# jabirali/bodge

Hardware: AMD Instinct MI355X
Metric: Chebyshev SpMV steps/s + achieved HBM GB/s, 4N×4N BdG H; free_energy wall-time (higher is better)
Workload: dtype f64

## Files before the change

bodge_amd/backend.py:

```python

from __future__ import annotations

import ctypes as C
import os

import numpy as np

LIBRARY_PATH = os.environ.get(
    "BODGE_AMD_LIBRARY", os.path.join(os.path.dirname(os.path.abspath(__file__)), "csrc", "libbodge_hip.so")
)

VEC_RADEMACHER = 0
VEC_Z4 = 1

_f64p = C.POINTER(C.c_double)
_i32p = C.POINTER(C.c_int32)
_i64p = C.POINTER(C.c_int64)
_u8p = C.POINTER(C.c_uint8)
_handle = C.c_void_p


class Perf(C.Structure):
    _fields_ = [
        ("kernel_ms", C.c_double),
        ("launches", C.c_int64),
        ("vector_steps", C.c_int64),
        ("bytes_per_launch", C.c_double),
        ("lanes_per_row", C.c_int32),
        ("vectors_per_launch", C.c_int32),
        ("grid", C.c_int32),
        ("lds_bytes", C.c_int32),
        ("pipelined", C.c_int32),
        ("real_arithmetic", C.c_int32),
        ("strip_rows", C.c_int32),
        ("ph_packed", C.c_int32),
        ("dict_blocks", C.c_int32),
        ("steps_per_launch", C.c_int32),
        ("rolling", C.c_int32),
        ("dict_skipped", C.c_int32),
        ("onsite_streamed", C.c_int32),
        ("streams", C.c_int32),
        ("bytes_moved", C.c_double),
        ("window_ms", C.c_double),
        ("sweeps", C.c_int64),
        ("persistent", C.c_int32),
        ("groups_per_launch", C.c_int32),
        ("clenshaw", C.c_int32),
        ("green", C.c_int32),
        ("green_ranges", C.c_int32),
        ("green_local", C.c_int32),
        ("apply", C.c_int32),
    ]


SIGNATURES = {
    "bdg_last_error": (C.c_char_p, []),
    "bdg_version": (C.c_char_p, []),
    "bdg_device_count": (C.c_int, [C.POINTER(C.c_int)]),
    "bdg_create": (C.c_int, [C.c_int, C.c_int64, C.c_int64, _i32p, _i32p, _f64p, C.POINTER(_handle)]),
    "bdg_create_slab": (
        C.c_int,
        [C.c_int, C.c_int64, C.c_int64, C.c_int64, _i32p, _i32p, _f64p, C.c_int64, C.POINTER(_handle)],
    ),
    "bdg_slab_set_exchange": (C.c_int, [_handle, _handle, C.c_int32, _i32p, _i64p, _i64p, _i64p, _i64p]),
    "bdg_group_create": (C.c_int, [C.POINTER(_handle), C.c_int32, C.POINTER(_handle)]),
    "bdg_group_destroy": (C.c_int, [_handle]),
    "bdg_group_dots_random": (
        C.c_int,
        [_handle, C.c_double, C.c_int32, C.c_int32, C.c_uint64, C.c_uint64, C.c_int32, _f64p, _f64p],
    ),
    "bdg_group_dots_unit": (C.c_int, [_handle, C.c_double, C.c_int32, C.c_int32, _i64p, _f64p, _f64p]),
    "bdg_destroy": (C.c_int, [_handle]),
    "bdg_spmv": (C.c_int, [_handle, _f64p, _f64p]),
    "bdg_cheb_dots_random": (
        C.c_int,
        [_handle, C.c_double, C.c_int32, C.c_int32, C.c_uint64, C.c_uint64, C.c_int32, _f64p, _f64p],
    ),
    "bdg_cheb_dots_unit": (C.c_int, [_handle, C.c_double, C.c_int32, C.c_int32, _i64p, _f64p, _f64p]),
    "bdg_cheb_moments": (
        C.c_int,
        [_handle, _handle, C.c_double, C.c_int32, C.c_int32, C.c_uint64, C.c_uint64, C.c_int32, _f64p],
    ),
    "bdg_fermi_blocks": (
        C.c_int,
# ... 127 lines not shown
```

bodge_amd/csrc/core.hpp:

```cpp
#pragma once

namespace {

thread_local std::string g_error;

int fail(int code, const char* fmt, ...) {
    char buf[512];
    va_list ap;
    va_start(ap, fmt);
    vsnprintf(buf, sizeof buf, fmt, ap);
    va_end(ap);
    g_error = buf;
    return code;
}

#define HIP_TRY(expr)                                                                   \
    do {                                                                                \
        hipError_t err__ = (expr);                                                      \
        if (err__ != hipSuccess)                                                        \
            return fail(err__ == hipErrorOutOfMemory ? BDG_ENOMEM : BDG_EDEVICE,        \
                        "%s failed: %s (%s:%d)", #expr, hipGetErrorString(err__),       \
                        __FILE__, __LINE__);                                            \
    } while (0)

// ... 118 lines not shown
    bool group_peer_access = true;
    hipStream_t comm_stream = nullptr;
    hipEvent_t ev_step_done = nullptr, ev_halo_ready = nullptr;
    DeviceBuffer<int> tiles_interior, tiles_boundary;
    int split_rows_per_tile = 0, n_interior = 0, n_boundary = 0;
    void* lanczos = nullptr;
    int max_row_blocks = 0;
    int64_t bandwidth = 0;
    int num_cus = 0;
    size_t lds_per_cu = 0;
    int lanes_override = 0;
    DeviceBuffer<int> indptr, indices;
    DeviceBuffer<double2> blocks;
    DeviceBuffer<double2> packed[4];
    bool is_real = false;
    bool is_ph = false;
    double gershgorin = 0.0;
    int n_unique = 0;
    int dict_skipped = 0;
    bool onsite_streamed = false;
    DeviceBuffer<double2> onsite[2];
    bool bonds_streamed = false;
    DeviceBuffer<double2> site_records[2];
    int site_records_plane[2] = {0, 0};
    DeviceBuffer<int> dict_ids;
    DeviceBuffer<unsigned> dict_ell;
    int dict_ell_words = 0;
    DeviceBuffer<int> dict_diagonal;
    DeviceBuffer<double2> dict_full;
    DeviceBuffer<double2> dict_table[4];
    DeviceBuffer<uint2> stencil;
    int stencil_state = 0;
    bool stencil_wrap_p = false, stencil_wrap_x = false;
    double* host_dots = nullptr;
    size_t host_dots_count = 0;
    int shape[3] = {0, 0, 0};
    struct TileOrder {
        int rows_per_tile = 0, strip_rows = 0;
        DeviceBuffer<int> ids;
    };
    std::vector<std::unique_ptr<TileOrder>> tile_orders;
    bdg_perf perf{};
};

namespace {
inline void release_side_sets(bdg_system* sys) {
    for (auto& side : sys->side_sets) {
        if (side->stream) (void)hipStreamSynchronize(side->stream);
        side->release_set();
    }
    sys->side_sets.clear();
}
}

struct bdg_comm {
    int device = 0;
    int n_ranks = 1, rank = 0;
    ncclComm_t comm = nullptr;
    hipStream_t stream = nullptr;
    DeviceBuffer<double> scratch;
};

struct bdg_group {
    std::vector<bdg_system*> members;
    std::vector<hipEvent_t> packed, copied;
    std::vector<hipEvent_t> stepped[2];
// ... 2 lines not shown
```

bodge_amd/csrc/plans.hpp:

```cpp
#pragma once

namespace {

using StepKernel = void (*)(bdg::StepArgs);

using bdg::ComplexMode;
using bdg::ComplexPHMode;
using bdg::RealMode;
using bdg::RealPHMode;

struct ModeInfo {
    int id;
    bool real, ph;
    int per_lane;
    int stride;
    double block_bytes;
    double entry_bytes;
};

ModeInfo mode_info(bool real, bool ph) {
    if (real && ph) return {3, true, true, RealPHMode::kVec, RealPHMode::kBlockStride, 100.0, 96.0};
    if (real) return {1, true, false, RealMode::kVec, RealMode::kBlockStride, 132.0, 96.0};
    if (ph) return {2, false, true, ComplexPHMode::kVec, ComplexPHMode::kBlockStride, 196.0, 192.0};
    return {0, false, false, ComplexMode::kVec, ComplexMode::kBlockStride, 260.0, 192.0};
// ... 388 lines not shown
}

SweepKernel sweep3_gen_kernel(const ModeInfo& mode, int lanes) {
    switch (mode.id) {
        case 1: return sweep3_gen_kernel_for<RealMode>(lanes);
        case 2: return sweep3_gen_kernel_for<ComplexPHMode>(lanes);
        case 3: return sweep3_gen_kernel_for<RealPHMode>(lanes);
    }
    return sweep3_gen_kernel_for<ComplexMode>(lanes);
}

template <typename Mode, int RL, int OS, int WAVES>
SweepKernel sweep3_streamed_pick(bool reverse, bool gen) {
    return gen ? bdg::cheb_sweep3<Mode, RL, false, true, OS, WAVES>
               : reverse ? bdg::cheb_sweep3<Mode, RL, true, false, OS, WAVES> : bdg::cheb_sweep3<Mode, RL, false, false, OS, WAVES>;
}
SweepKernel sweep3_streamed_kernel(const ModeInfo& mode, int lanes, int waves, bool reverse, bool gen, bool bonds = false) {
    if (!mode.ph) return nullptr;
    if (bonds) {
        if (mode.real) return lanes == 4 && waves == 4 ? sweep3_streamed_pick<RealPHMode, 4, 2, 4>(reverse, gen) : nullptr;
        return lanes == 4 && waves == 7 ? sweep3_streamed_pick<ComplexPHMode, 4, 2, 7>(reverse, gen) : nullptr;
    }
    if (mode.real) {
        if (lanes == 4 && waves == 4) return sweep3_streamed_pick<RealPHMode, 4, 1, 4>(reverse, gen);
        if (lanes == 2 && waves == 4) return sweep3_streamed_pick<RealPHMode, 2, 1, 4>(reverse, gen);
        if (lanes == 2 && waves == 7) return sweep3_streamed_pick<RealPHMode, 2, 1, 7>(reverse, gen);
        return nullptr;
    }
    if (lanes == 4 && waves == 4) return sweep3_streamed_pick<ComplexPHMode, 4, 1, 4>(reverse, gen);
    if (lanes == 2 && waves == 7) return sweep3_streamed_pick<ComplexPHMode, 2, 1, 7>(reverse, gen);
    return nullptr;
}

size_t sweep3_lds_bytes(const bdg_system* sys, const ModeInfo& mode, int lanes, int waves) {
    size_t bytes = (size_t)sys->n_unique * mode.stride * sizeof(double2) +
                   (size_t)sys->n_unique * (mode.id == 0 ? 4 : mode.id == 3 ? 1 : 2) * sizeof(double2) +
                   (size_t)sys->n_unique * (mode.id == 3 ? RealPHMode::kSingletSlots : 0) * sizeof(double2);
    size_t per_wave = (size_t)3 * bdg::kWave * 4 * sizeof(double2);
    if (sys->onsite_streamed) {
        const int stride = sys->bonds_streamed ? (mode.real ? bdg::sweep3_record_stride<RealPHMode, 2>() : bdg::sweep3_record_stride<ComplexPHMode, 2>())
                                               : (mode.real ? bdg::sweep3_record_stride<RealPHMode, 1>() : bdg::sweep3_record_stride<ComplexPHMode, 1>());
        per_wave += (size_t)3 * (bdg::kWave / lanes) * stride * sizeof(double2);
    }
    return bytes + (size_t)waves * per_wave;
}

int streamed_waves_for(const bdg_system* sys, const ModeInfo& mode, int lanes) {
    if (!sys->onsite_streamed || !mode.ph) return 0;
    int best = 0, best_resident = 0;
    for (int waves : {4, 7}) {
        if (!sweep3_streamed_kernel(mode, lanes, waves, false, false, sys->bonds_streamed)) continue;
        const size_t lds = sweep3_lds_bytes(sys, mode, lanes, waves);
        if (lds > sys->lds_per_cu) continue;
        const int resident = waves * (int)std::min<size_t>(waves > 4 ? 1 : 2, sys->lds_per_cu / lds);
        if (resident > best_resident) best = waves, best_resident = resident;
    }
    return best;
}

SweepKernel sweep3_kernel(const ModeInfo& mode, int lanes, bool reverse) {
    switch (mode.id) {
        case 1: return sweep3_kernel_for<RealMode>(lanes, reverse);
        case 2: return sweep3_kernel_for<ComplexPHMode>(lanes, reverse);
        case 3: return sweep3_kernel_for<RealPHMode>(lanes, reverse);
    }
    return sweep3_kernel_for<ComplexMode>(lanes, reverse);
}

using MarchKernel = void (*)(bdg::MarchArgs);
template <typename Mode>
MarchKernel march3_kernel_for(int lanes) {
    switch (lanes) {
        case 2: return bdg::cheb_march3<Mode, 2, 0>;
        case 4: return bdg::cheb_march3<Mode, 4, 0>;
    }
    return nullptr;
}
MarchKernel march3_kernel(const ModeInfo& mode, int lanes, bool streamed, bool bonds) {
    if (streamed) {
        if (!mode.ph || lanes != 4) return nullptr;
        if (bonds) return mode.real ? bdg::cheb_march3<RealPHMode, 4, 2> : nullptr;
        return mode.real ? bdg::cheb_march3<RealPHMode, 4, 1> : bdg::cheb_march3<ComplexPHMode, 4, 1>;
    }
    switch (mode.id) {
        case 1: return march3_kernel_for<RealMode>(lanes);
        case 2: return march3_kernel_for<ComplexPHMode>(lanes);
        case 3: return march3_kernel_for<RealPHMode>(lanes);
    }
    return march3_kernel_for<ComplexMode>(lanes);
}

struct SweepPlan {
    int lanes = bdg::kSweepLanes;
    int depth = 2;
    SweepKernel kernel = nullptr, kernel_reverse = nullptr;
    SweepKernel kernel_gen = nullptr;
    MarchKernel march = nullptr;
    int march_grid = 0;
    int grid = 0;
    int wg_waves = bdg::kSweepWaves;
    size_t lds_bytes = 0;
    bdg::SweepArgs args{};
    int waves = 0;
    int whole_segs = 1;
    int segments_for(int planes) const {
        if (planes >= args.lx) return whole_segs;
        return std::max(1, std::min(choose_segments(args.n_cols, planes, waves, 2 * depth, 2), planes / 2));
    }
};

constexpr int64_t kSweepMinSites = 150000;
constexpr int64_t kSweepMinSitesWide = 90000;
constexpr int64_t kRollMinSites = 600000;
constexpr int64_t kSweepTwoLaneSites = 250000;

int ensure_stencil(bdg_system* sys, int* kind) {
    *kind = 0;
    const int64_t plane = (int64_t)sys->shape[1] * sys->shape[2];
    if (sys->stencil_state == 0) {
        sys->stencil_state = -1;
        sys->stencil_lo_base = sys->stencil_hi_base = -1;
        const bool shaped = plane >= 2 * bdg::kSweepOwned && sys->shape[0] >= 8 &&
                            (int64_t)sys->shape[0] * plane == sys->nb;
        const bool three_d = sys->shape[1] > 1 && sys->shape[2] > 1;
        bool slab_ok = sys->ncols == sys->nb;
        if (!slab_ok && shaped && three_d) {
            slab_ok = true;
            const int64_t lx = sys->shape[0];
            int64_t lo = -1, hi = -1;
            for (const auto& ref : sys->halo_refs) {
                const int64_t x = ref.first / plane, p = ref.first % plane, base = (int64_t)ref.second - p;
                if (x == 0 && (lo < 0 || lo == base)) lo = base;
                else if (x == lx - 1 && (hi < 0 || hi == base)) hi = base;
                else slab_ok = false;
            }
            for (int64_t base : {lo, hi})
                if (base >= 0 && (base < sys->nb || base + plane > sys->ncols)) slab_ok = false;
            if (slab_ok) {
                sys->stencil_lo_base = (int)lo;
                sys->stencil_hi_base = (int)hi;
            }
        }
        if (shaped && slab_ok && sys->n_unique > 0 && sys->n_unique < (int)bdg::kNoBlock &&
            sys->max_row_blocks <= (three_d ? 7 : 5) && sys->nnzb > 0 && !(three_d && sys->onsite_streamed)) {
            if (int rc = sys->stencil.reserve((size_t)sys->nb)) return rc;
            DeviceBuffer<int> bad;
            if (int rc = bad.reserve(3)) return rc;
            int host_bad[3] = {1, 0, 0};
            auto body = [&]() -> int {
                HIP_TRY(hipMemsetAsync(bad.ptr, 0, 3 * sizeof(int), sys->stream));
                const unsigned grid = (unsigned)std::min<int64_t>(4096, (sys->nb + 255) / 256);
                if (three_d)
                    bdg::build_stencil3<<<grid, 256, 0, sys->stream>>>(sys->indptr.ptr, sys->dict_ids.ptr,
                                                                        sys->dict_diagonal.ptr, (int)sys->nb, (int)plane,
                                                                        sys->shape[2], sys->stencil_lo_base, sys->stencil_hi_base,
                                                                        sys->stencil.ptr, bad.ptr);
                else
                    bdg::build_stencil<<<grid, 256, 0, sys->stream>>>(sys->indptr.ptr, sys->dict_ids.ptr,
                                                                       sys->dict_diagonal.ptr, (int)sys->nb, (int)plane,
                                                                       sys->bonds_streamed ? 2 : sys->onsite_streamed ? 1 : 0,
                                                                       sys->stencil.ptr, bad.ptr);
                HIP_TRY(hipGetLastError());
                HIP_TRY(hipMemcpyAsync(host_bad, bad.ptr, 3 * sizeof(int), hipMemcpyDeviceToHost, sys->stream));
                HIP_TRY(hipStreamSynchronize(sys->stream));
                return BDG_OK;
            };
            const int rc = body();
            bad.release();
            if (rc) return rc;
            if (host_bad[0] == 0) {
                sys->stencil_state = three_d ? 2 : 1;
                sys->stencil_wrap_p = host_bad[1] != 0;
                sys->stencil_wrap_x = host_bad[2] != 0;
            } else {
                sys->stencil.release();
            }
        }
    }
    *kind = std::max(0, sys->stencil_state);
    return BDG_OK;
}

inline int64_t plane_sites(const bdg_system* sys) { return (int64_t)sys->shape[1] * sys->shape[2]; }

int sweep_wanted(bdg_system* sys, bool col_scalars, int* kind, bool wide_call = false) {
    *kind = 0;
    const char* env = knob::raw("BODGE_AMD_SWEEP");
    if ((env && env[0] == '0') || col_scalars) return BDG_OK;
    const bool slab = !sys->peers.empty() || sys->ncols != sys->nb;
    if (slab && (sys->slab_comm || sys->group_rows == 0)) return BDG_OK;
    const bool forced = env && env[0] == '1';
    const int64_t lattice_rows = std::max(sys->nb, sys->group_rows);
    const int64_t min_2d = wide_call ? kSweepMinSitesWide : kSweepMinSites;
    if (!forced && lattice_rows < std::min(min_2d, kRollMinSites)) return BDG_OK;
    const char* dict_env = knob::raw("BODGE_AMD_DICT");
    if (dict_env && dict_env[0] == '0') return BDG_OK;
    if (int rc = ensure_stencil(sys, kind)) return rc;
    if (slab && *kind != 2) *kind = 0;
    if (!forced && lattice_rows < (*kind == 2 ? kRollMinSites : min_2d)) *kind = 0;
    return BDG_OK;
}

int make_sweep_plan(bdg_system* sys, const ModeInfo& mode, int lanes, int depth, SweepPlan* plan, int share = 1) {
    plan->lanes = lanes;
    plan->depth = depth;
    const bool streamed = sys->onsite_streamed, bonds = sys->bonds_streamed;
    const int wg_waves = streamed ? streamed_waves_for(sys, mode, lanes) : bdg::kSweepWaves;
    if (streamed && (depth != 3 || wg_waves == 0))
        return fail(BDG_EINVAL, "streamed on-site blocks need the three-step sweep, particle-hole packed blocks and a lane count whose ring of records fits the LDS (%d lanes do not)", lanes);
    plan->wg_waves = wg_waves;
    plan->kernel = streamed ? sweep3_streamed_kernel(mode, lanes, wg_waves, false, false, bonds)
                            : depth == 3 ? sweep3_kernel(mode, lanes, false) : sweep_kernel(mode, lanes, false);
    plan->kernel_reverse = streamed ? sweep3_streamed_kernel(mode, lanes, wg_waves, true, false, bonds)
                                    : depth == 3 ? sweep3_kernel(mode, lanes, true) : sweep_kernel(mode, lanes, true);
    plan->kernel_gen = streamed ? sweep3_streamed_kernel(mode, lanes, wg_waves, false, true, bonds) : depth == 3 ? sweep3_gen_kernel(mode, lanes) : nullptr;
    if (!plan->kernel) return fail(BDG_EINVAL, "the sweep kernel has 1, 2 or 4 lanes per site, not %d", lanes);
    const size_t table = (size_t)sys->n_unique * mode.stride * sizeof(double2);
    if (table > table_limit(sys)) return fail(BDG_EINVAL, "block table too large for the sweep kernel");
    if (depth == 3) {
        plan->lds_bytes = sweep3_lds_bytes(sys, mode, lanes, wg_waves);
    } else {
        plan->lds_bytes = table + (size_t)bdg::kSweepWaves * depth * bdg::kWave * 4 * sizeof(double2);
    }
    if (plan->lds_bytes > 64 * 1024)
        for (SweepKernel k : {plan->kernel, plan->kernel_reverse, plan->kernel_gen})
            if (k) HIP_TRY(hipFuncSetAttribute(reinterpret_cast<const void*>(k), hipFuncAttributeMaxDynamicSharedMemorySize,
                                        (int)plan->lds_bytes));
    plan->march = depth == 3 && wg_waves == bdg::kWavesPerBlock &&
                          (size_t)sys->ncols * lanes * 4 * sizeof(double2) < ((size_t)1 << 31) && sys->ncols == sys->nb
                      ? march3_kernel(mode, lanes, streamed, bonds) : nullptr;
    if (plan->march && plan->lds_bytes > 64 * 1024)
        HIP_TRY(hipFuncSetAttribute(reinterpret_cast<const void*>(plan->march), hipFuncAttributeMaxDynamicSharedMemorySize,
                                    (int)plan->lds_bytes));
    int per_cu = 0;
    HIP_TRY(hipOccupancyMaxActiveBlocksPerMultiprocessor(&per_cu, reinterpret_cast<const void*>(plan->kernel),
                                                         wg_waves * bdg::kWave, plan->lds_bytes));
    per_cu = std::max(1, std::min(per_cu, wg_waves > 4 ? 1 : 2 * bdg::kWavesPerBlock / bdg::kSweepWaves));
    if (const char* cap = knob::raw("BODGE_AMD_BLOCKS_PER_CU")) per_cu = std::max(1, atoi(cap));
    const int64_t plane = (int64_t)sys->shape[1] * sys->shape[2];
    bdg::SweepArgs& a = plan->args;
    a = bdg::SweepArgs{};
    a.stencil = sys->stencil.ptr;
    if (int rc = ensure_dict_table(sys, mode, &a.dict_table)) return rc;
    if (bonds) {
        if (int rc = ensure_site_records(sys, (int)plane, mode.real, &a.onsite)) return rc;
    } else if (streamed) {
        if (int rc = ensure_onsite(sys, mode.real, &a.onsite)) return rc;
    }
    a.n_unique = sys->n_unique;
    a.nb = (int)sys->nb;
    a.plane = (int)plane;
    a.lx = sys->shape[0];
    const int owned = depth == 3 ? bdg::sweep3_owned(lanes) : bdg::sweep_owned(lanes);
// ... 194 lines not shown
```

bodge_amd/csrc/recurrence.hpp:

```cpp
#pragma once

namespace {

constexpr int kMarchAborted = -77;

struct Batch {
    bdg_system* sys = nullptr;
    StreamSet* ss = nullptr;
    int next = 0;
    int stream_share = 1;
    StepPlan plan;
    bdg::StepArgs args{};
    bool real = false;
    bool alternate = false;
    int64_t band_lo = -1, band_hi = -1;
    int plane_lo = -1, plane_hi = -1;
    ModeInfo mode{};
    int rl = 0, rv = 0, n_active = 0, n_steps = 0, chunk = 1, strip_rows = 0;
    size_t width = 0, per_step = 0, vec_count = 0;
    double scale = 1.0;
    double2* cur = nullptr;
    double2* prev = nullptr;
    float kernel_ms = 0.f;
    int n_chunks = 0;
// ... 575 lines not shown
            sys->march_seen[0] = 0;
            (void)hipMemsetAsync(sys->march_gave_up.ptr, 0, sizeof(unsigned), sys->stream);
            (void)hipStreamSynchronize(sys->stream);
            sys->march_off = true;
            return kMarchAborted;
        }
        const double* host = sys->host_dots + (size_t)slot * host_stride;
        if (march_follower) n_chunks = 0;
        for (int c = 0; c < n_chunks; ++c) {
            float ms = 0.f;
            HIP_TRY(hipEventElapsedTime(&ms, ss->ev_pool[2 * (ev_base + c)], ss->ev_pool[2 * (ev_base + c) + 1]));
            kernel_ms += ms;
        }
        for (int n = 0; n < n_steps; ++n)
            for (int r = 0; r < n_active; ++r) {
                double& d = d_out[(size_t)n * ld + col0 + r];
                double& e = e_out[(size_t)n * ld + col0 + r];
                const double dv = host[(size_t)n * width + 2 * r], ev = host[(size_t)n * width + 2 * r + 1];
                d = accumulate ? d + dv : dv;
                e = accumulate ? e + ev : ev;
            }
        bdg_perf& p = sys->perf;
        if (first_batch) p = bdg_perf{};
        p.kernel_ms += kernel_ms;
        p.launches += sweep ? n_launches : n_steps;
        p.bytes_moved += bytes_moved;
        p.window_ms = p.kernel_ms;
        p.streams = 1;
        p.vector_steps += (int64_t)n_steps * n_active;
        p.bytes_per_launch = sweep  ? sweep_bytes(sys, mode, rl)
                             : roll ? roll_bytes(sys, mode, rl)
                                    : algorithmic_bytes(sys, rv, mode, plan.dictionary);
        p.steps_per_launch = sweep ? splan.depth : 1;
        p.persistent = march ? 1 : 0;
        p.sweeps += march ? sweeps_counted : sweep ? n_launches : 0;
        p.rolling = roll ? 1 : 0;
        p.dict_skipped = sys->dict_skipped;
        p.onsite_streamed = sweep && sys->onsite_streamed ? (sys->bonds_streamed ? 2 : 1) : 0;
        p.lanes_per_row = rl;
        p.vectors_per_launch = rv;
        p.real_arithmetic = real ? 1 : 0;
        p.ph_packed = mode.ph ? 1 : 0;
        p.dict_blocks = plan.dictionary ? sys->n_unique : 0;
        p.strip_rows = strip_rows;
        p.grid = march ? splan.march_grid : launch_grid;
        p.lds_bytes = (int32_t)(sweep ? splan.lds_bytes : roll ? rplan.lds_bytes : plan.lds_footprint);
        p.pipelined = plan.pipelined ? 1 : 0;
        return BDG_OK;
    }
};

int march_run(Batch* const* list, int count) {
    Batch& lead = *list[0];
    bdg_system* sys = lead.sys;
    HIP_TRY(hipSetDevice(sys->device));
    hipStream_t st = lead.ss->stream;
    const bdg::SweepArgs& geo = lead.splan.args;
    const int units = geo.n_cols * geo.n_segs;
    for (int g = 0; g < count; ++g) {
        Batch& b = *list[g];
        if (!b.march || b.next != lead.next || b.n_steps != lead.n_steps || b.rl != lead.rl || b.mode.id != lead.mode.id ||
            b.splan.args.n_segs != geo.n_segs || b.chunk != lead.chunk)
            return fail(BDG_EINVAL, "lane groups of one persistent launch must share plan and progress");
        b.march_follower = g > 0;
        b.work_stream = st;
        if (g > 0) {
// ... 441 lines not shown
```

bodge_amd/csrc/sweep.hpp:

```cpp
#pragma once

#include "kernels.hpp"

namespace bdg {

constexpr int kSweepLanes = 4;
constexpr int kSweepSlots = kWave / kSweepLanes;
constexpr int kSweepOwned = kSweepSlots - 4;
constexpr int sweep_owned(int rl) { return kWave / rl - 4; }
constexpr unsigned kNoBlock = 0xFFu;

struct SweepArgs {
    const uint2* stencil;
    const void* dict_table;
    int n_unique;
    const double2* onsite;
    const double2* cur;
    const double2* prev;
    double2* out1;
    double2* out2;
    double* partial1;
    double* partial2;
    double coef1, coef2;
    int nb;
// ... 21 lines not shown
    const int lx = nb / plane;
    for (int i = blockIdx.x * blockDim.x + threadIdx.x; i < nb; i += gridDim.x * blockDim.x) {
        unsigned id[5] = {kNoBlock, kNoBlock, kNoBlock, kNoBlock, kNoBlock};
        unsigned mask = 0;
        const int p = i % plane, x = i / plane;
        bool ok = true;
        for (int k = indptr[i]; k < indptr[i + 1]; ++k) {
            const unsigned w = (unsigned)words[k];
            const int off = (int)(w & 0xFFFFFFu) - i;
            int slot = -1;
            if (off == -plane) slot = 0;
            else if (off == -1 && p >= 1) slot = 1;
            else if (off == 0) slot = 2;
            else if (off == 1 && p <= plane - 2) slot = 3;
            else if (off == plane) slot = 4;
            else if (off == plane - 1 && p == 0) {
                slot = 1;
                atomicOr(bad + 1, 1);
            } else if (off == -(plane - 1) && p == plane - 1) {
                slot = 3;
                atomicOr(bad + 1, 1);
            } else if (off == (lx - 1) * plane && x == 0) {
                slot = 0;
                atomicOr(bad + 2, 1);
            } else if (off == -(lx - 1) * plane && x == lx - 1) {
                slot = 4;
                atomicOr(bad + 2, 1);
            }
            if (slot < 0 || (w >> 24) == kNoBlock) ok = false;
            else if (onsite_streamed == 2 || (onsite_streamed && slot == 2)) id[slot] = 0;
            else {
                id[slot] = w >> 24;
                if (diagonal[w >> 24] == 1) mask |= 1u << slot;
                if (diagonal[w >> 24] == 2 && slot != 2) mask |= 32u << slot;
            }
        }
        if (!ok) atomicOr(bad, 1);
        stencil[i] = make_uint2(id[0] | (id[1] << 8) | (id[2] << 16) | (id[3] << 24), id[4] | (mask << 8));
    }
}

__global__ void pack_site_records(const int* __restrict__ indptr, const int* __restrict__ indices,
                                  const double2* __restrict__ blocks, int nb, int plane, int real_out, double2* __restrict__ out) {
    const int lx = nb / plane;
    for (int i = blockIdx.x * blockDim.x + threadIdx.x; i < nb; i += gridDim.x * blockDim.x) {
        const double2 zero = make_double2(0.0, 0.0);
        double2 rec[14] = {zero, zero, zero, zero, zero, zero, zero, zero, zero, zero, zero, zero, zero, zero};
        const int p = i % plane, x = i / plane;
        for (int k = indptr[i]; k < indptr[i + 1]; ++k) {
            const double2* blk = blocks + (size_t)k * 16;
            const int off = indices[k] - i;
            int slot = -1;
            if (off == -plane) slot = 0;
            else if (off == -1 && p >= 1) slot = 1;
            else if (off == 0) slot = 2;
            else if (off == 1 && p <= plane - 2) slot = 3;
            else if (off == plane) slot = 4;
            else if (off == plane - 1 && p == 0) slot = 1;
            else if (off == -(plane - 1) && p == plane - 1) slot = 3;
            else if (off == (lx - 1) * plane && x == 0) slot = 0;
            else if (off == -(lx - 1) * plane && x == lx - 1) slot = 4;
            const int bond = slot < 2 ? slot : slot - 1;
            if (slot == 2 && real_out) {
                rec[0] = make_double2(blk[0].x, blk[1].x);
                rec[1] = make_double2(blk[5].x, 0.0);
                rec[2] = make_double2(blk[2].x, blk[3].x);
// ... 288 lines not shown
#define BDG_SWEEP_BUFFER_OPS 1
#endif
__device__ __forceinline__ __amdgpu_buffer_rsrc_t sweep_plane_rsrc(const void* buf, size_t byte_offset, int bytes) {
    const uint64_t base = reinterpret_cast<uint64_t>(buf) + byte_offset;
    const uint32_t lo = __builtin_amdgcn_readfirstlane((uint32_t)base), hi = __builtin_amdgcn_readfirstlane((uint32_t)(base >> 32));
    return __builtin_amdgcn_make_buffer_rsrc(reinterpret_cast<void*>(((uint64_t)hi << 32) | lo), 0, bytes, kRawBufferFlags);
}

struct Sweep3Gen {
    uint64_t key0 = 0, key1 = 0;
    bool on0 = false, on1 = false;
};
template <typename Mode>
__device__ inline Sweep3Gen sweep3_gen_keys(uint64_t seed, uint64_t first_id, int active, int r) {
    Sweep3Gen g;
    const int v0 = Mode::kVec == 2 ? 2 * r : r;
    g.on0 = v0 < active;
    g.on1 = Mode::kVec == 2 && v0 + 1 < active;
    g.key0 = vector_key(seed, first_id + v0);
    g.key1 = vector_key(seed, first_id + v0 + 1);
    return g;
}

struct Sweep3Task {
    const double2* cur;
    const double2* prev;
    double2* out1;
    double2* out2;
    double coef1;
    int steps;
    int discard;
};

template <typename Mode, int RL, bool GEN, int OS, bool WT>
__device__ __forceinline__ void sweep3_unit(const SweepArgs& a, const Sweep3Task& t, const Sweep3Lds& w, const Sweep3Gen& gen, int lane,
                                            int seg, int col, bool rev, double (&dot1)[4], double (&dot2)[4], double (&dot3)[4]) {
    constexpr int SLOTS = kWave / RL;
    constexpr int OWNED3 = SLOTS - 6;
    constexpr int STRIDE = Mode::kBlockStride;
    constexpr int RING = sweep3_ring_slots<Mode, OS>(SLOTS);
    constexpr int RSTRIDE = sweep3_record_stride<Mode, OS>();
    constexpr int DSL = Mode::kDiagSlots;
    const int s = lane / RL;
    const int r = lane % RL;
    double2* const lds = w.table;
    double2* const diag = w.diag;
    [[maybe_unused]] double2* const singlet = w.singlet;
    double2* const row_0 = w.row_0;
    double2* const row_1 = w.row_1;
    double2* const row_2 = w.row_2;
    [[maybe_unused]] double2* const os_ring = w.os_ring;
    const double2 zero = make_double2(0.0, 0.0);
    const size_t nb = (size_t)a.nb;
    const int steps = t.steps;
    const bool nt_prev = a.stream & 1, nt_cur = a.stream & 4;
    [[maybe_unused]] const bool nt_store = a.stream & 2;
    [[maybe_unused]] const uint64_t gen_key0 = gen.key0, gen_key1 = gen.key1;
    [[maybe_unused]] const bool gen_on0 = gen.on0, gen_on1 = gen.on1;

    const int x0 = a.x_lo + (int)(((int64_t)(a.x_hi - a.x_lo) * seg) / a.n_segs);
    const int x1 = a.x_lo + (int)(((int64_t)(a.x_hi - a.x_lo) * (seg + 1)) / a.n_segs);
    const int p = col * OWNED3 - 3 + s;
    const bool inside = p >= 0 && p < a.plane;
    const bool valid = inside || a.wrap_p;
    const int pw = inside ? p : ((p % a.plane) + a.plane) % a.plane;
    const bool ok1 = valid && s >= 1 && s <= SLOTS - 2;
    const bool ok2 = valid && s >= 2 && s <= SLOTS - 3;
// ... 138 lines not shown
        double2 x[4];
        [[maybe_unused]] const double2* rec = nullptr;
        if constexpr (OS != 0) rec = ring_entry(kk) + s * RSTRIDE;
        auto bond = [&](int slot, const double2 v[4]) {
            if constexpr (OS == 2) {
                if (id_of(w, slot) != kNoBlock) Mode::mac_bond(acc, rec + Mode::kOnsiteSlots + Mode::kBondSlots * (slot < 2 ? slot : slot - 1), v);
            } else {
                mac(w, slot, v, acc);
            }
        };
        if (rev) bond(0, after);
        else bond(0, before);
        if (id_of(w, 1) != kNoBlock) {
#pragma unroll
            for (int be = 0; be < 4; ++be) x[be] = row[SHARE_SLOT(lane - RL, be)];
            bond(1, x);
        }
        if constexpr (OS != 0) {
#if !(BDG_OS_EXPERIMENT & 4)
            if (id_of(w, 2) != kNoBlock) Mode::mac_onsite(acc, rec, mid);
#endif
        } else {
            mac(w, 2, mid, acc);
        }
        if (id_of(w, 3) != kNoBlock) {
#pragma unroll
            for (int be = 0; be < 4; ++be) x[be] = row[SHARE_SLOT(lane + RL, be)];
            bond(3, x);
        }
        if (rev) bond(4, before);
        else bond(4, after);
    };

    constexpr int OSL = OS != 0 ? (SLOTS * sweep3_onsite_pieces<Mode, OS>() + kWave - 1) / kWave : 1;
    [[maybe_unused]] auto load_onsite = [&](int k, bool wanted, double2 out[OSL]) {
        if constexpr (OS != 0) {
            constexpr int PIECES = sweep3_record_slots<Mode, OS>();
            k = ring(act(k));
#pragma unroll
            for (int j = 0; j < OSL; ++j) {
                const int e = lane + j * kWave, slot = e / PIECES, part = e - slot * PIECES;
                const int pe = col * OWNED3 - 3 + slot;
                const bool in_e = pe >= 0 && pe < a.plane;
                const int pwe = in_e ? pe : ((pe % a.plane) + a.plane) % a.plane;
                out[j] = zero;
                {
                    const bool there = wanted && k >= 0 && k < a.lx;
                    const __amdgpu_buffer_rsrc_t rsrc = sweep_plane_rsrc(a.onsite, there ? (size_t)k * a.plane * PIECES * sizeof(double2) : 0,
                                                                         there ? a.plane * PIECES * (int)sizeof(double2) : 0);
                    const int piece_bytes = slot < SLOTS && (in_e || a.wrap_p) ? (pwe * PIECES + part) * (int)sizeof(double2) : kBufferOutOfRange;
                    out[j] = __builtin_bit_cast(double2, __builtin_amdgcn_raw_buffer_load_b128(rsrc, piece_bytes, 0, 0));
                }
            }
        }
    };
    [[maybe_unused]] auto put_onsite = [&](int kk, const double2 v[OSL]) {
        if constexpr (OS != 0) {
            constexpr int PIECES = sweep3_record_slots<Mode, OS>();
            double2* dst = ring_entry(kk);
#pragma unroll
            for (int j = 0; j < OSL; ++j) {
                const int e = lane + j * kWave, slot = e / PIECES, part = e - slot * PIECES;
                if (slot < SLOTS) dst[slot * RSTRIDE + part] = v[j];
            }
        }
    };

    double2 cn_m[4], buf_a[4], buf_b[4], pv[4], c1_m[4], c2_m[4];
    cur_plane(k_first - 1, valid, cn_m);
    cur_plane(k_first, valid, buf_a);
    cur_plane(k_first + 1, valid, buf_b);
    load_plane(t.prev, nt_prev, k_first, !GEN && ok1 && t.prev != nullptr, pv);
    uint2 ids_0 = load_ids(k_first), ids_1 = make_uint2(0xFFFFFFFFu, 0xFFu), ids_2 = ids_1;
#pragma unroll
    for (int al = 0; al < 4; ++al) c1_m[al] = c2_m[al] = zero;
    put_own(row_1, c1_m);
    put_own(row_2, c1_m);
    if constexpr (OS != 0) {
        double2 first_os[OSL];
        load_onsite(k_first, true, first_os);
        put_onsite(k_first, first_os);
    }

    auto iterate = [&](int k, double2 (&centre)[4], const double2 (&after)[4]) {
        const bool more = k < k_last;
        const uint2 nx_ids = load_ids(k + 1, more);
        put_own(row_0, centre);
        wave_sync();
        cur_plane(k + 2, valid && more, centre);

        double2 new1[4], new2[4];
#pragma unroll
        for (int al = 0; al < 4; ++al) new1[al] = new2[al] = zero;
        if (ok1 && in_lattice(k)) {
            double2 acc[4], mid[4];
#pragma unroll
            for (int al = 0; al < 4; ++al) acc[al] = zero;
            own_of(row_0, mid);
            apply(ids_0, cn_m, row_0, mid, after, acc, k);
#pragma unroll
            for (int al = 0; al < 4; ++al) {
                new1[al].x = fma(t.coef1, acc[al].x, -pv[al].x);
                new1[al].y = fma(t.coef1, acc[al].y, -pv[al].y);
            }
            if (owned && k >= x0 && k < x1) {
#pragma unroll
                for (int al = 0; al < 4; ++al) Mode::dots(dot1, mid[al], new1[al]);
                if (steps == 1) store_plane(t.out2, k, new1);
                if (steps == 2) store_plane(t.out1, k, new1);
            }
        }
        load_plane(t.prev, nt_prev, k + 1, !GEN && ok1 && more && t.prev != nullptr, pv);

        if (steps >= 2 && ok2 && in_lattice(k - 1) && k - 1 >= x0 - (steps - 2) && k - 1 < x1 + (steps - 2)) {
            double2 acc[4], mid[4];
#pragma unroll
            for (int al = 0; al < 4; ++al) acc[al] = zero;
            own_of(row_1, mid);
            apply(ids_1, c1_m, row_1, mid, new1, acc, k - 1);
#pragma unroll
            for (int al = 0; al < 4; ++al) {
                new2[al].x = fma(a.coef2, acc[al].x, -cn_m[al].x);
                new2[al].y = fma(a.coef2, acc[al].y, -cn_m[al].y);
            }
            if (owned && k - 1 >= x0 && k - 1 < x1) {
#pragma unroll
                for (int al = 0; al < 4; ++al) Mode::dots(dot2, mid[al], new2[al]);
                if (steps == 2) store_plane(t.out2, k - 1, new2);
                if (steps == 3) store_plane(t.out1, k - 1, new2);
            }
        }

        [[maybe_unused]] double2 nx_os[OSL];
#if BDG_OS_EXPERIMENT & 1
        load_onsite(k + 1, false, nx_os);
#else
        load_onsite(k + 1, more, nx_os);
#endif

        if (steps >= 3 && owned && k - 2 >= x0 && k - 2 < x1) {
            double2 acc[4], mid[4], new3[4];
#pragma unroll
            for (int al = 0; al < 4; ++al) acc[al] = zero;
            own_of(row_2, mid);
            apply(ids_2, c2_m, row_2, mid, new2, acc, k - 2);
#pragma unroll
            for (int al = 0; al < 4; ++al) {
                new3[al].x = fma(a.coef2, acc[al].x, -c1_m[al].x);
                new3[al].y = fma(a.coef2, acc[al].y, -c1_m[al].y);
                Mode::dots(dot3, mid[al], new3[al]);
            }
            store_plane(t.out2, k - 2, new3);
        }

        wave_sync();
        own_of(row_0, cn_m);
        own_of(row_1, c1_m);
        own_of(row_2, c2_m);
        wave_sync();
        put_own(row_1, new1);
        put_own(row_2, new2);
#if !(BDG_OS_EXPERIMENT & 2)
        put_onsite(k + 1, nx_os);
#endif
        ids_2 = ids_1;
        ids_1 = ids_0;
        ids_0 = nx_ids;
    };
    for (int k = k_first; k <= k_last; k += 2) {
        iterate(k, buf_a, buf_b);
        if (k + 1 <= k_last) iterate(k + 1, buf_b, buf_a);
    }
}

template <typename Mode, int OS, int THREADS = kBlockThreads>
__device__ inline Sweep3Lds sweep3_stage_lds(double2* lds, const SweepArgs& a, int slots, int wave) {
    constexpr int SPB = Mode::kSlotsPerBlock;
    constexpr int STRIDE = Mode::kBlockStride;
    constexpr int DSL = Mode::kDiagSlots;
    const int ring = sweep3_ring_slots<Mode, OS>(slots);
    const double2* table = static_cast<const double2*>(a.dict_table);
    for (int e = threadIdx.x; e < a.n_unique * SPB; e += THREADS)
        lds[(e / SPB) * STRIDE + (e % SPB)] = table[e];
    constexpr int SSL = Mode::kSingletSlots;
    Sweep3Lds w;
    w.table = lds;
    w.diag = lds + a.n_unique * STRIDE;
    w.singlet = w.diag + a.n_unique * DSL;
    w.row_0 = w.singlet + a.n_unique * SSL + wave * (3 * kWave * 4 + ring);
    w.row_1 = w.row_0 + kWave * 4;
    w.row_2 = w.row_1 + kWave * 4;
    w.os_ring = w.row_2 + kWave * 4;
    __syncthreads();
    for (int id = threadIdx.x; id < a.n_unique; id += THREADS) {
        Mode::pack_diag(w.diag + id * DSL, lds + id * STRIDE);
        if constexpr (SSL > 0) Mode::pack_singlet(w.singlet + id * SSL, lds + id * STRIDE);
    }
    __syncthreads();
    return w;
}

template <typename Mode, int RL, bool REV, bool GEN = false, int OS = 0, int WAVES = kWavesPerBlock>
__global__ __launch_bounds__(WAVES * kWave, WAVES > 4 ? 1 : 2) void cheb_sweep3(SweepArgs a) {
    extern __shared__ double2 lds[];
    const int lane = threadIdx.x & (kWave - 1);
    const int wave = __builtin_amdgcn_readfirstlane(threadIdx.x / kWave);
    const Sweep3Lds w = sweep3_stage_lds<Mode, OS, WAVES * kWave>(lds, a, kWave / RL, wave);

    const int n_units = a.n_cols * a.n_segs;
    const int xcd = blockIdx.x & 7;
    const int u_lo = (int)(((int64_t)n_units * xcd) >> 3);
    const int u_hi = (int)(((int64_t)n_units * (xcd + 1)) >> 3);
    const int waves_per_xcd = (gridDim.x >> 3) * WAVES;

    double dot1[4] = {0.0, 0.0, 0.0, 0.0}, dot2[4] = {0.0, 0.0, 0.0, 0.0}, dot3[4] = {0.0, 0.0, 0.0, 0.0};
    Sweep3Gen gen;
    if constexpr (GEN) gen = sweep3_gen_keys<Mode>(a.gen_seed, a.gen_first_id, a.gen_active, lane % RL);

    const Sweep3Task task{a.cur, a.prev, a.out1, a.out2, a.coef1, a.steps, a.discard};
    for (int u = u_lo + (int)(blockIdx.x >> 3) * WAVES + wave; u < u_hi; u += waves_per_xcd) {
        const int seg = u / a.n_cols, col = u - seg * a.n_cols;
        const bool rev = REV != (bool)(a.zigzag & seg & 1);
        sweep3_unit<Mode, RL, GEN, OS, false>(a, task, w, gen, lane, seg, col, rev, dot1, dot2, dot3);
    }

    const int steps = a.steps;
    __syncthreads();
    sweep_reduce_dots<Mode, RL, WAVES>(dot1, reinterpret_cast<double*>(lds), a.partial1, lane, wave);
    if (steps >= 2) {
        __syncthreads();
        sweep_reduce_dots<Mode, RL, WAVES>(dot2, reinterpret_cast<double*>(lds), a.partial2, lane, wave);
    }
    if (steps >= 3) {
        __syncthreads();
        sweep_reduce_dots<Mode, RL, WAVES>(dot3, reinterpret_cast<double*>(lds), a.partial3, lane, wave);
    }
}

constexpr int kMarchGroups = 4;
constexpr int kMarchMaxLevels = 24;
constexpr int kMarchCounterWords = 32;

struct MarchGroup {
    double2* buf[4];
    double* partial;
    unsigned long long gen_first_id;
    int gen_active;
    int pad;
};

struct MarchArgs {
    SweepArgs base;
    MarchGroup group[kMarchGroups];
    int n_groups;
    int n_levels;
    int last_steps;
    int discard_last;
    int first_is_start;
    int gen;
    int rev0;
    int units;
    unsigned long long per_step;
    unsigned* sync;
    unsigned flags_at;
    unsigned timeout_ticks;
    unsigned* gave_up;
    int fixed;
    int debug;
    int poll_sleep;
// ... 384 lines not shown
```

include/bodge_hip.h:

```cpp
#ifndef BODGE_HIP_H
#define BODGE_HIP_H

#include <stdint.h>

#ifdef __cplusplus
extern "C" {
#endif

#define BDG_OK 0
#define BDG_EINVAL (-1)
#define BDG_EDEVICE (-2)
#define BDG_ENOMEM (-3)
#define BDG_ELIBRARY (-4)

#define BDG_VEC_RADEMACHER 0
#define BDG_VEC_Z4 1

typedef struct bdg_system bdg_system;
typedef struct bdg_comm bdg_comm;
typedef struct bdg_group bdg_group;

typedef struct bdg_perf {
    double kernel_ms;
    int64_t launches;
    int64_t vector_steps;
    double bytes_per_launch;
    int32_t lanes_per_row;
    int32_t vectors_per_launch;
    int32_t grid;
    int32_t lds_bytes;
    int32_t pipelined;
    int32_t real_arithmetic;
    int32_t strip_rows;
    int32_t ph_packed;
    int32_t dict_blocks;
    int32_t steps_per_launch;
    int32_t rolling;
    int32_t dict_skipped;
    int32_t onsite_streamed;
    int32_t streams;
    double bytes_moved;
    double window_ms;
    int64_t sweeps;
    int32_t persistent;
    int32_t groups_per_launch;
    int32_t clenshaw;
    int32_t green;
    int32_t green_ranges;
    int32_t green_local;
    int32_t apply;
} bdg_perf;

const char* bdg_last_error(void);
const char* bdg_version(void);

int bdg_device_count(int* count);

int bdg_create(int device, int64_t nb, int64_t nnzb, const int32_t* indptr,
               const int32_t* indices, const double* data, bdg_system** out);
int bdg_destroy(bdg_system* sys);

int bdg_create_slab(int device, int64_t nb, int64_t ncols, int64_t nnzb, const int32_t* indptr,
                    const int32_t* indices, const double* data, int64_t row_offset,
                    bdg_system** out);
int bdg_slab_set_exchange(bdg_system* sys, bdg_comm* comm, int32_t n_peers, const int32_t* peer_rank,
                          const int64_t* send_count, const int64_t* send_rows,
                          const int64_t* recv_col, const int64_t* recv_count);
int bdg_group_create(bdg_system** members, int32_t n_members, bdg_group** out);
int bdg_group_destroy(bdg_group* group);
int bdg_group_dots_random(bdg_group* group, double scale, int32_t n_steps, int32_t n_vectors,
                          uint64_t seed, uint64_t first_vec_id, int32_t vec_kind,
                          double* d_out, double* e_out);
int bdg_group_dots_unit(bdg_group* group, double scale, int32_t n_steps, int32_t n_vectors,
                        const int64_t* rows, double* d_out, double* e_out);

int bdg_spmv(bdg_system* sys, const double* x, double* y);

int bdg_cheb_dots_random(bdg_system* sys, double scale, int32_t n_steps, int32_t n_vectors,
                         uint64_t seed, uint64_t first_vec_id, int32_t vec_kind,
                         double* d_out, double* e_out);
int bdg_cheb_dots_unit(bdg_system* sys, double scale, int32_t n_steps, int32_t n_vectors,
                       const int64_t* rows, double* d_out, double* e_out);

// ... 72 lines not shown
```

Measured before the change: 109,900.

## Add branch-free straight-line stencil products for plain 2D sweep kernels

```diff
diff --git a/bodge_amd/backend.py b/bodge_amd/backend.py
--- a/bodge_amd/backend.py
+++ b/bodge_amd/backend.py
@@ -50,6 +50,7 @@
         ("green_ranges", C.c_int32),
         ("green_local", C.c_int32),
         ("apply", C.c_int32),
+        ("straight_line", C.c_int32),
     ]
 
 
diff --git a/bodge_amd/csrc/core.hpp b/bodge_amd/csrc/core.hpp
--- a/bodge_amd/csrc/core.hpp
+++ b/bodge_amd/csrc/core.hpp
@@ -174,6 +174,7 @@
     DeviceBuffer<uint2> stencil;
     int stencil_state = 0;
     bool stencil_wrap_p = false, stencil_wrap_x = false;
+    bool stencil_plain = false;
     double* host_dots = nullptr;
     size_t host_dots_count = 0;
     int shape[3] = {0, 0, 0};
diff --git a/bodge_amd/csrc/plans.hpp b/bodge_amd/csrc/plans.hpp
--- a/bodge_amd/csrc/plans.hpp
+++ b/bodge_amd/csrc/plans.hpp
@@ -444,10 +444,11 @@
     return nullptr;
 }
 
-size_t sweep3_lds_bytes(const bdg_system* sys, const ModeInfo& mode, int lanes, int waves) {
-    size_t bytes = (size_t)sys->n_unique * mode.stride * sizeof(double2) +
-                   (size_t)sys->n_unique * (mode.id == 0 ? 4 : mode.id == 3 ? 1 : 2) * sizeof(double2) +
-                   (size_t)sys->n_unique * (mode.id == 3 ? RealPHMode::kSingletSlots : 0) * sizeof(double2);
+size_t sweep3_lds_bytes(const bdg_system* sys, const ModeInfo& mode, int lanes, int waves, bool pad = false) {
+    const size_t entries = (size_t)sys->n_unique + (pad ? 1 : 0);
+    size_t bytes = entries * mode.stride * sizeof(double2) +
+                   entries * (mode.id == 0 ? 4 : mode.id == 3 ? 1 : 2) * sizeof(double2) +
+                   entries * (mode.id == 3 ? RealPHMode::kSingletSlots : 0) * sizeof(double2);
     size_t per_wave = (size_t)3 * bdg::kWave * 4 * sizeof(double2);
     if (sys->onsite_streamed) {
         const int stride = sys->bonds_streamed ? (mode.real ? bdg::sweep3_record_stride<RealPHMode, 2>() : bdg::sweep3_record_stride<ComplexPHMode, 2>())
@@ -479,6 +480,17 @@
     return sweep3_kernel_for<ComplexMode>(lanes, reverse);
 }
 
+template <typename Mode, int RL>
+SweepKernel sweep3h_pick(int form) {
+    return form == 2 ? bdg::cheb_sweep3h<Mode, RL, false, true>
+           : form == 1 ? bdg::cheb_sweep3h<Mode, RL, true, false> : bdg::cheb_sweep3h<Mode, RL, false, false>;
+}
+SweepKernel sweep3h_kernel(const ModeInfo& mode, int lanes, int form) {
+    if (!mode.ph || (lanes != 2 && lanes != 4)) return nullptr;
+    if (mode.real) return lanes == 2 ? sweep3h_pick<RealPHMode, 2>(form) : sweep3h_pick<RealPHMode, 4>(form);
+    return lanes == 2 ? sweep3h_pick<ComplexPHMode, 2>(form) : sweep3h_pick<ComplexPHMode, 4>(form);
+}
+
 using MarchKernel = void (*)(bdg::MarchArgs);
 template <typename Mode>
 MarchKernel march3_kernel_for(int lanes) {
@@ -507,6 +519,7 @@
     int depth = 2;
     SweepKernel kernel = nullptr, kernel_reverse = nullptr;
     SweepKernel kernel_gen = nullptr;
+    int straight = 0;
     MarchKernel march = nullptr;
     int march_grid = 0;
     int grid = 0;
@@ -557,10 +570,10 @@
             sys->max_row_blocks <= (three_d ? 7 : 5) && sys->nnzb > 0 && !(three_d && sys->onsite_streamed)) {
             if (int rc = sys->stencil.reserve((size_t)sys->nb)) return rc;
             DeviceBuffer<int> bad;
-            if (int rc = bad.reserve(3)) return rc;
-            int host_bad[3] = {1, 0, 0};
+            if (int rc = bad.reserve(4)) return rc;
+            int host_bad[4] = {1, 0, 0, 1};
             auto body = [&]() -> int {
-                HIP_TRY(hipMemsetAsync(bad.ptr, 0, 3 * sizeof(int), sys->stream));
+                HIP_TRY(hipMemsetAsync(bad.ptr, 0, 4 * sizeof(int), sys->stream));
                 const unsigned grid = (unsigned)std::min<int64_t>(4096, (sys->nb + 255) / 256);
                 if (three_d)
                     bdg::build_stencil3<<<grid, 256, 0, sys->stream>>>(sys->indptr.ptr, sys->dict_ids.ptr,
@@ -573,7 +586,7 @@
                                                                        sys->bonds_streamed ? 2 : sys->onsite_streamed ? 1 : 0,
                                                                        sys->stencil.ptr, bad.ptr);
                 HIP_TRY(hipGetLastError());
-                HIP_TRY(hipMemcpyAsync(host_bad, bad.ptr, 3 * sizeof(int), hipMemcpyDeviceToHost, sys->stream));
+                HIP_TRY(hipMemcpyAsync(host_bad, bad.ptr, 4 * sizeof(int), hipMemcpyDeviceToHost, sys->stream));
                 HIP_TRY(hipStreamSynchronize(sys->stream));
                 return BDG_OK;
             };
@@ -584,6 +597,7 @@
                 sys->stencil_state = three_d ? 2 : 1;
                 sys->stencil_wrap_p = host_bad[1] != 0;
                 sys->stencil_wrap_x = host_bad[2] != 0;
+                sys->stencil_plain = !three_d && !sys->onsite_streamed && host_bad[3] == 0;
             } else {
                 sys->stencil.release();
             }
@@ -626,11 +640,19 @@
     plan->kernel_reverse = streamed ? sweep3_streamed_kernel(mode, lanes, wg_waves, true, false, bonds)
                                     : depth == 3 ? sweep3_kernel(mode, lanes, true) : sweep_kernel(mode, lanes, true);
     plan->kernel_gen = streamed ? sweep3_streamed_kernel(mode, lanes, wg_waves, false, true, bonds) : depth == 3 ? sweep3_gen_kernel(mode, lanes) : nullptr;
+    plan->straight = 0;
+    if (const char* env = knob::raw("BODGE_AMD_SWEEP_STRAIGHT");
+        depth == 3 && !streamed && sys->stencil_plain && !(env && env[0] == '0') && sweep3h_kernel(mode, lanes, 0)) {
+        plan->straight = 1;
+        plan->kernel = sweep3h_kernel(mode, lanes, 0);
+        plan->kernel_reverse = sweep3h_kernel(mode, lanes, 1);
+        plan->kernel_gen = sweep3h_kernel(mode, lanes, 2);
+    }
     if (!plan->kernel) return fail(BDG_EINVAL, "the sweep kernel has 1, 2 or 4 lanes per site, not %d", lanes);
     const size_t table = (size_t)sys->n_unique * mode.stride * sizeof(double2);
     if (table > table_limit(sys)) return fail(BDG_EINVAL, "block table too large for the sweep kernel");
     if (depth == 3) {
-        plan->lds_bytes = sweep3_lds_bytes(sys, mode, lanes, wg_waves);
+        plan->lds_bytes = sweep3_lds_bytes(sys, mode, lanes, wg_waves, plan->straight != 0);
     } else {
         plan->lds_bytes = table + (size_t)bdg::kSweepWaves * depth * bdg::kWave * 4 * sizeof(double2);
     }
diff --git a/bodge_amd/csrc/recurrence.hpp b/bodge_amd/csrc/recurrence.hpp
--- a/bodge_amd/csrc/recurrence.hpp
+++ b/bodge_amd/csrc/recurrence.hpp
@@ -631,6 +631,7 @@
                              : roll ? roll_bytes(sys, mode, rl)
                                     : algorithmic_bytes(sys, rv, mode, plan.dictionary);
         p.steps_per_launch = sweep ? splan.depth : 1;
+        p.straight_line = sweep && !march && splan.straight != 0 ? 1 : 0;
         p.persistent = march ? 1 : 0;
         p.sweeps += march ? sweeps_counted : sweep ? n_launches : 0;
         p.rolling = roll ? 1 : 0;
diff --git a/bodge_amd/csrc/sweep.hpp b/bodge_amd/csrc/sweep.hpp
--- a/bodge_amd/csrc/sweep.hpp
+++ b/bodge_amd/csrc/sweep.hpp
@@ -77,6 +77,7 @@
             else {
                 id[slot] = w >> 24;
                 if (diagonal[w >> 24] == 1) mask |= 1u << slot;
+                else if (slot != 2) atomicOr(bad + 3, 1);
                 if (diagonal[w >> 24] == 2 && slot != 2) mask |= 32u << slot;
             }
         }
@@ -431,7 +432,7 @@
     int discard;
 };
 
-template <typename Mode, int RL, bool GEN, int OS, bool WT>
+template <typename Mode, int RL, bool GEN, int OS, bool WT, bool STRAIGHT = false>
 __device__ __forceinline__ void sweep3_unit(const SweepArgs& a, const Sweep3Task& t, const Sweep3Lds& w, const Sweep3Gen& gen, int lane,
                                             int seg, int col, bool rev, double (&dot1)[4], double (&dot2)[4], double (&dot3)[4]) {
     constexpr int SLOTS = kWave / RL;
@@ -636,6 +637,44 @@
         else bond(4, after);
     };
 
+    [[maybe_unused]] auto apply_straight = [&](uint2 w, const double2 before[4], const double2* row, const double2 mid[4],
+                                               const double2 after[4], double2 acc[4]) {
+        static_assert(!STRAIGHT || OS == 0, "the straight-line products read every block from the table");
+        const unsigned none = (unsigned)a.n_unique;
+        unsigned at[5];
+#pragma unroll
+        for (int slot = 0; slot < 5; ++slot) at[slot] = min(id_of(w, slot), none);
+        const unsigned at_fb = rev ? none : at[0], at_fa = rev ? at[0] : none;
+        const unsigned at_la = rev ? none : at[4], at_lb = rev ? at[4] : none;
+        double2 lo[4], hi[4], d_fb[DSL], d_fa[DSL], d_lo[DSL], d_hi[DSL], d_la[DSL], d_lb[DSL];
+        constexpr int NOS = Mode::kSlotsPerBlock;
+        double2 os[NOS];
+#pragma unroll
+        for (int be = 0; be < 4; ++be) lo[be] = row[SHARE_SLOT(lane - RL, be)];
+#pragma unroll
+        for (int e = 0; e < DSL; ++e) d_fb[e] = diag[at_fb * DSL + e], d_fa[e] = diag[at_fa * DSL + e], d_lo[e] = diag[at[1] * DSL + e];
+#pragma unroll
+        for (int e = 0; e < NOS; ++e) os[e] = lds[at[2] * STRIDE + e];
+        constexpr bool OS_AHEAD = NOS <= 6;
+        Mode::mac_diag_compact(acc, d_fb, before);
+        Mode::mac_diag_compact(acc, d_fa, after);
+        Mode::mac_diag_compact(acc, d_lo, lo);
+#pragma unroll
+        for (int be = 0; be < 4; ++be) hi[be] = row[SHARE_SLOT(lane + RL, be)];
+#pragma unroll
+        for (int e = 0; e < DSL; ++e) d_hi[e] = diag[at[3] * DSL + e], d_la[e] = diag[at_la * DSL + e], d_lb[e] = diag[at_lb * DSL + e];
+        if constexpr (OS_AHEAD) Mode::mac_row(acc, os, mid);
+        else Mode::mac_row(acc, lds + at[2] * STRIDE, mid);
+        Mode::mac_diag_compact(acc, d_hi, hi);
+        if constexpr (OS_AHEAD) {
+            Mode::mac_diag_compact(acc, d_la, after);
+            Mode::mac_diag_compact(acc, d_lb, before);
+        } else {
+            Mode::mac_diag_compact(acc, diag + at_la * DSL, after);
+            Mode::mac_diag_compact(acc, diag + at_lb * DSL, before);
+        }
+    };
+
     constexpr int OSL = OS != 0 ? (SLOTS * sweep3_onsite_pieces<Mode, OS>() + kWave - 1) / kWave : 1;
     [[maybe_unused]] auto load_onsite = [&](int k, bool wanted, double2 out[OSL]) {
         if constexpr (OS != 0) {
@@ -701,7 +740,8 @@
 #pragma unroll
             for (int al = 0; al < 4; ++al) acc[al] = zero;
             own_of(row_0, mid);
-            apply(ids_0, cn_m, row_0, mid, after, acc, k);
+            if constexpr (STRAIGHT) apply_straight(ids_0, cn_m, row_0, mid, after, acc);
+            else apply(ids_0, cn_m, row_0, mid, after, acc, k);
 #pragma unroll
             for (int al = 0; al < 4; ++al) {
                 new1[al].x = fma(t.coef1, acc[al].x, -pv[al].x);
@@ -721,7 +761,8 @@
 #pragma unroll
             for (int al = 0; al < 4; ++al) acc[al] = zero;
             own_of(row_1, mid);
-            apply(ids_1, c1_m, row_1, mid, new1, acc, k - 1);
+            if constexpr (STRAIGHT) apply_straight(ids_1, c1_m, row_1, mid, new1, acc);
+            else apply(ids_1, c1_m, row_1, mid, new1, acc, k - 1);
 #pragma unroll
             for (int al = 0; al < 4; ++al) {
                 new2[al].x = fma(a.coef2, acc[al].x, -cn_m[al].x);
@@ -747,7 +788,8 @@
 #pragma unroll
             for (int al = 0; al < 4; ++al) acc[al] = zero;
             own_of(row_2, mid);
-            apply(ids_2, c2_m, row_2, mid, new2, acc, k - 2);
+            if constexpr (STRAIGHT) apply_straight(ids_2, c2_m, row_2, mid, new2, acc);
+            else apply(ids_2, c2_m, row_2, mid, new2, acc, k - 2);
 #pragma unroll
             for (int al = 0; al < 4; ++al) {
                 new3[al].x = fma(a.coef2, acc[al].x, -c1_m[al].x);
@@ -777,7 +819,7 @@
     }
 }
 
-template <typename Mode, int OS, int THREADS = kBlockThreads>
+template <typename Mode, int OS, int THREADS = kBlockThreads, bool PAD = false>
 __device__ inline Sweep3Lds sweep3_stage_lds(double2* lds, const SweepArgs& a, int slots, int wave) {
     constexpr int SPB = Mode::kSlotsPerBlock;
     constexpr int STRIDE = Mode::kBlockStride;
@@ -786,17 +828,20 @@
     const double2* table = static_cast<const double2*>(a.dict_table);
     for (int e = threadIdx.x; e < a.n_unique * SPB; e += THREADS)
         lds[(e / SPB) * STRIDE + (e % SPB)] = table[e];
+    const int entries = a.n_unique + (PAD ? 1 : 0);
+    if constexpr (PAD)
+        for (int e = threadIdx.x; e < SPB; e += THREADS) lds[a.n_unique * STRIDE + e] = make_double2(0.0, 0.0);
     constexpr int SSL = Mode::kSingletSlots;
     Sweep3Lds w;
     w.table = lds;
-    w.diag = lds + a.n_unique * STRIDE;
-    w.singlet = w.diag + a.n_unique * DSL;
-    w.row_0 = w.singlet + a.n_unique * SSL + wave * (3 * kWave * 4 + ring);
+    w.diag = lds + entries * STRIDE;
+    w.singlet = w.diag + entries * DSL;
+    w.row_0 = w.singlet + entries * SSL + wave * (3 * kWave * 4 + ring);
     w.row_1 = w.row_0 + kWave * 4;
     w.row_2 = w.row_1 + kWave * 4;
     w.os_ring = w.row_2 + kWave * 4;
     __syncthreads();
-    for (int id = threadIdx.x; id < a.n_unique; id += THREADS) {
+    for (int id = threadIdx.x; id < entries; id += THREADS) {
         Mode::pack_diag(w.diag + id * DSL, lds + id * STRIDE);
         if constexpr (SSL > 0) Mode::pack_singlet(w.singlet + id * SSL, lds + id * STRIDE);
     }
@@ -804,12 +849,12 @@
     return w;
 }
 
-template <typename Mode, int RL, bool REV, bool GEN = false, int OS = 0, int WAVES = kWavesPerBlock>
-__global__ __launch_bounds__(WAVES * kWave, WAVES > 4 ? 1 : 2) void cheb_sweep3(SweepArgs a) {
+template <typename Mode, int RL, bool REV, bool GEN, int OS, int WAVES, bool STRAIGHT>
+__device__ __forceinline__ void sweep3_launch(const SweepArgs& a) {
     extern __shared__ double2 lds[];
     const int lane = threadIdx.x & (kWave - 1);
     const int wave = __builtin_amdgcn_readfirstlane(threadIdx.x / kWave);
-    const Sweep3Lds w = sweep3_stage_lds<Mode, OS, WAVES * kWave>(lds, a, kWave / RL, wave);
+    const Sweep3Lds w = sweep3_stage_lds<Mode, OS, WAVES * kWave, STRAIGHT>(lds, a, kWave / RL, wave);
 
     const int n_units = a.n_cols * a.n_segs;
     const int xcd = blockIdx.x & 7;
@@ -825,7 +870,7 @@
     for (int u = u_lo + (int)(blockIdx.x >> 3) * WAVES + wave; u < u_hi; u += waves_per_xcd) {
         const int seg = u / a.n_cols, col = u - seg * a.n_cols;
         const bool rev = REV != (bool)(a.zigzag & seg & 1);
-        sweep3_unit<Mode, RL, GEN, OS, false>(a, task, w, gen, lane, seg, col, rev, dot1, dot2, dot3);
+        sweep3_unit<Mode, RL, GEN, OS, false, STRAIGHT>(a, task, w, gen, lane, seg, col, rev, dot1, dot2, dot3);
     }
 
     const int steps = a.steps;
@@ -839,6 +884,16 @@
         __syncthreads();
         sweep_reduce_dots<Mode, RL, WAVES>(dot3, reinterpret_cast<double*>(lds), a.partial3, lane, wave);
     }
+}
+
+template <typename Mode, int RL, bool REV, bool GEN = false, int OS = 0, int WAVES = kWavesPerBlock>
+__global__ __launch_bounds__(WAVES * kWave, WAVES > 4 ? 1 : 2) void cheb_sweep3(SweepArgs a) {
+    sweep3_launch<Mode, RL, REV, GEN, OS, WAVES, false>(a);
+}
+
+template <typename Mode, int RL, bool REV, bool GEN = false>
+__global__ __launch_bounds__(kWavesPerBlock * kWave, 2) void cheb_sweep3h(SweepArgs a) {
+    sweep3_launch<Mode, RL, REV, GEN, 0, kWavesPerBlock, true>(a);
 }
 
 constexpr int kMarchGroups = 4;
diff --git a/include/bodge_hip.h b/include/bodge_hip.h
--- a/include/bodge_hip.h
+++ b/include/bodge_hip.h
@@ -49,6 +49,7 @@
     int32_t green_ranges;
     int32_t green_local;
     int32_t apply;
+    int32_t straight_line;
 } bdg_perf;
 
 const char* bdg_last_error(void);
```

Result: faster. 111,900, median of 6 (+1.8%).
